# jchristopherson/nonlin

Measured on AMD Instinct MI355X. Metric: LM iterations/sec on m=4096,n=256 fp64; FD-Jacobian GB/s vs HBM peak, higher is better.
Workload: dtype f64

## Files before the change

### nonlin_amd/csrc/nlh_core.hip

```cpp
#include "nlh_internal.h"
#include "nlh_kernels_model.h"
#include "nlh_qrx.h"

int ensure(nlh_handle *h, DevBuf &b, size_t bytes)
{
    if (bytes <= b.bytes && b.p) return 0;
    if (b.p) { hipFree(b.p); b.p = nullptr; b.bytes = 0; }
    size_t want = bytes < 256 ? 256 : bytes;
    hipError_t e = hipMalloc(&b.p, want);
    if (e != hipSuccess) { h->err = std::string("hipMalloc: ") + hipGetErrorString(e); return NLH_OUT_OF_MEMORY_ERROR; }
    b.bytes = want;
    bool known = false;
    for (auto *q : h->bufs) if (q == &b) known = true;
    if (!known) h->bufs.push_back(&b);
    return 0;
}

bool lds_fits(const void *kernel, size_t dyn)
{
    static std::mutex mu;
    static std::vector<std::pair<const void *, size_t>> statics;
    size_t st = 0;
    {
        std::lock_guard<std::mutex> g(mu);
        auto it = std::find_if(statics.begin(), statics.end(), [&](const std::pair<const void *, size_t> &e) { return e.first == kernel; });
        if (it != statics.end()) st = it->second;
        else {
            hipFuncAttributes a;
            st = hipFuncGetAttributes(&a, kernel) == hipSuccess ? a.sharedSizeBytes : (size_t)NLH_LDS_MAX;
            statics.emplace_back(kernel, st);
        }
    }
    return st + dyn <= (size_t)NLH_LDS_MAX;
}

int ensure_staging(nlh_handle *h, size_t bytes)
{
    if (bytes <= h->staging_bytes) return 0;
    if (h->staging) hipHostFree(h->staging);
    h->staging = nullptr; h->staging_bytes = 0;
    if (hipHostMalloc(&h->staging, bytes, hipHostMallocDefault) != hipSuccess) { h->err = "hipHostMalloc (staging)"; return NLH_OUT_OF_MEMORY_ERROR; }
    h->staging_bytes = bytes;
    return 0;
}

int ensure_pinned(nlh_handle *h, size_t bytes)
{
    if (bytes <= h->pinned_bytes) return 0;
    if (h->pinned) hipHostFree(h->pinned);
    h->pinned = nullptr; h->pinned_bytes = 0;
    hipError_t e = hipHostMalloc(&h->pinned, bytes, hipHostMallocDefault);
    if (e != hipSuccess) { h->err = std::string("hipHostMalloc: ") + hipGetErrorString(e); return NLH_OUT_OF_MEMORY_ERROR; }
    h->pinned_bytes = bytes;
    return 0;
}

static const char *k_names[NLH_K_COUNT] = {
    "k_dq_residual", "k_dq_panel", "k_fd_jacobian", "k_gram_mfma", "k_gram_reduce", "k_jtf",
    "k_chol_factor", "k_lmpar", "k_qr_factor", "k_lm_update", "k_lu_factor", "k_dq_jacobian", "k_qrx_pass",
    "k_qrx_pivot", "k_polyroots", "k_covar"};

void timing_flush(nlh_handle *h)
{
    if (h->pending.empty()) return;
    hipStreamSynchronize(h->stream);
    for (auto &pr : h->pending) {
        float t = 0.f;
        if (hipEventElapsedTime(&t, pr.a, pr.b) == hipSuccess) h->ms[pr.kid] += (double)t;
        h->launches[pr.kid] += 1;
        if (pr.kid == h->sample_kid) h->samples.push_back(t);
        h->pool.push_back(pr.a);
        h->pool.push_back(pr.b);
    }
    h->pending.clear();
}

hipEvent_t ev_get(nlh_handle *h)
{
    if (!h->pool.empty()) { hipEvent_t e = h->pool.back(); h->pool.pop_back(); return e; }
    hipEvent_t e;
    hipEventCreate(&e);
    return e;
}
void nlh_default_options(nlh_options *o)
{
    o->max_evals = 100;
    o->ftol = 1.0e-8;
    o->xtol = 1.0e-12;
    o->gtol = 1.0e-12;
    o->print_status = 0;
    o->factor = 100.0;
    o->use_line_search = 1;
    o->ls_max_evals = 100;
    o->ls_alpha = 1.0e-4;
    o->ls_factor = 0.1;
    o->factor_policy = NLH_FACTOR_EXACT;
    o->ne_pivot_tol = 1.0e-4;
    o->fuse_fd = 1;
    o->sub_batches = 0;
}

int nlh_device_count(void)
{
    int n = 0;
    if (hipGetDeviceCount(&n) != hipSuccess) return 0;
    return n;
}

const char *nlh_version(void) { return "nonlin_hip 0.1 (gfx950)"; }

int nlh_create(nlh_handle **out, int32_t device, void *hip_stream)
{
    if (!out) return NLH_ERR_BAD_HANDLE;
    *out = nullptr;
    if (nlh_device_count() <= 0) return NLH_ERR_NO_DEVICE;
    if (hipSetDevice(device) != hipSuccess) return NLH_ERR_NO_DEVICE;
    nlh_handle *h = new nlh_handle();
    h->device = device;
    h->stream = (hipStream_t)hip_stream;
    const int lds_max = NLH_LDS_MAX;
    qrx_init_device();
    nlh_lm_init_device(lds_max);
    nlh_square_init_device(lds_max);
    nlh_cls_init_device(lds_max);
    nlh_bfgs_init_device(lds_max);
    nlh_poly_init_device(lds_max);
    nlh_polyroots_init_device(lds_max);
    nlh_covar_init_device(lds_max);
    nlh_devfcn_init_device(lds_max);
    nlh_expr_init_device(lds_max);
    (void)hipFuncSetAttribute((const void *)k_dq_residual<RB>, hipFuncAttributeMaxDynamicSharedMemorySize, lds_max);
    (void)hipFuncSetAttribute((const void *)k_dq_residual2<RB / 2>, hipFuncAttributeMaxDynamicSharedMemorySize, lds_max);
    (void)hipGetLastError();
    *out = h;
    return 0;
}

void nlh_destroy(nlh_handle *h)
{
    if (!h) return;
    for (auto *wk : h->workers) nlh_destroy(wk);
    h->workers.clear();
    hipSetDevice(h->device);
    hipStreamSynchronize(h->stream);
    timing_flush(h);
    for (auto e : h->pool) hipEventDestroy(e);
    for (auto *b : h->bufs) if (b->p) hipFree(b->p);
    if (h->pinned) hipHostFree(h->pinned);
    if (h->staging) hipHostFree(h->staging);
    if (h->lu_side) { hipStreamSynchronize(h->lu_side); hipStreamDestroy(h->lu_side); }
    if (h->lu_panel_done) hipEventDestroy(h->lu_panel_done);
    for (auto e : h->lu_bulk_done) if (e) hipEventDestroy(e);
    if (h->own_stream) hipStreamDestroy(h->stream);
    delete h;
}

const char *nlh_last_error(const nlh_handle *h) { return h ? h->err.c_str() : "null handle"; }

void nlh_timing_enable(nlh_handle *h, int32_t on)
{
    if (!h) return;
    h->timing = on == 0 ? 0u : on == 1 ? 0xffffffffu : ((uint32_t)on >> 1);
}
void nlh_timing_reset(nlh_handle *h)
{
    if (!h) return;
    timing_flush(h);
    for (int k = 0; k < NLH_K_COUNT; ++k) { h->ms[k] = 0; h->launches[k] = 0; }
    h->samples.clear();
}
int64_t nlh_timing_samples(nlh_handle *h, int32_t kid, float *out_ms, int64_t cap)
{
    if (!h) return NLH_ERR_BAD_HANDLE;
    if (kid != h->sample_kid) {
        timing_flush(h);
        h->sample_kid = kid;
        h->samples.clear();
        return 0;
    }
    timing_flush(h);
    const int64_t cnt = (int64_t)h->samples.size();
    for (int64_t i = 0; i < cnt && i < cap; ++i) out_ms[i] = h->samples[(size_t)i];
    return cnt;
}
int nlh_timing_get(nlh_handle *h, int32_t kid, double *total_ms, int64_t *launches)
{
    if (!h || kid < 0 || kid >= NLH_K_COUNT) return NLH_ERR_BAD_HANDLE;
    timing_flush(h);
    if (total_ms) *total_ms = h->ms[kid];
    if (launches) *launches = h->launches[kid];
    return 0;
}
const char *nlh_kernel_name(int32_t kid) { return (kid >= 0 && kid < NLH_K_COUNT) ? k_names[kid] : "?"; }




__device__ __forceinline__ double sm64_u(uint64_t seed, uint64_t k)
{
    uint64_t z = seed + (k + 1ULL) * 0x9E3779B97F4A7C15ULL;
    z = (z ^ (z >> 30)) * 0xBF58476D1CE4E5B9ULL;
    z = (z ^ (z >> 27)) * 0x94D049BB133111EBULL;
    z ^= z >> 31;
    return (double)(z >> 11) * 0x1.0p-53;
}

__global__ void k_gen_A(int m, int n, uint64_t seed0, uint64_t stride, int square_shift, double *A, double *xtrue)
{
    const int p = blockIdx.y;
    const uint64_t seed = seed0 + (uint64_t)p * stride;
    const size_t mn = (size_t)m * n;
    const double rs = sqrt((double)n);
    for (size_t e = (size_t)blockIdx.x * blockDim.x + threadIdx.x; e < mn + (size_t)n; e += (size_t)gridDim.x * blockDim.x) {
        const double u = 2.0 * sm64_u(seed, e) - 1.0;
        if (e < mn) {
            double v = u / rs;
            const size_t i = e % m, j = e / m;
            if (square_shift && i == j) v = 2.0 + v;
            A[(size_t)p * mn + e] = v;
        } else {
            xtrue[(size_t)p * n + (e - mn)] = u;
        }
    }
}

__global__ void k_gen_bx(int m, int n, uint64_t seed0, uint64_t stride, double sigma, double spread, double *b,
                         const double *xtrue, double *x0)
{
    const int p = blockIdx.y;
    const uint64_t seed = seed0 + (uint64_t)p * stride;
    const size_t base = (size_t)m * n + (size_t)n;
    for (size_t e = (size_t)blockIdx.x * blockDim.x + threadIdx.x; e < (size_t)m + n; e += (size_t)gridDim.x * blockDim.x) {
        const double u = 2.0 * sm64_u(seed, base + e) - 1.0;
        if (e < (size_t)m) b[(size_t)p * m + e] = b[(size_t)p * m + e] + sigma * u;
        else x0[(size_t)p * n + (e - m)] = xtrue[(size_t)p * n + (e - m)] + spread * u;
    }
}


void launch_dq_residual(nlh_handle *h, int nprob, int m, int n, const double *A, const double *b,
                               double gamma, const double *x, double *f, double *part,
                               const LmState *st, int want)
{
    Timed t(h, NLH_K_DQ_RESIDUAL);
    size_t sh = sizeof(double) * (size_t)(n + 32);
    const bool vec2 = (m % 2 == 0) && ((((uintptr_t)A | (uintptr_t)b | (uintptr_t)f) & 15) == 0);
    const int nblk = (m + RB - 1) / RB;
    for (int p0 = 0; p0 < nprob; p0 += NLH_MAX_LOCKSTEP) {
        const int cnt = std::min<int>(NLH_MAX_LOCKSTEP, nprob - p0);
        dim3 grid(nblk, cnt);
        const double *Ap = A + (size_t)p0 * m * n, *bp = b + (size_t)p0 * m, *xp = x + (size_t)p0 * n;
        double *fp = f + (size_t)p0 * m, *pp = part ? part + (size_t)p0 * nblk * 2 : nullptr;
        const LmState *sp = st ? st + p0 : nullptr;
        if (vec2)
            hipLaunchKernelGGL(k_dq_residual2<RB / 2>, grid, dim3(RB / 2), sh, h->stream, m, n, Ap, bp, gamma, xp, fp, pp, sp, want);
        else
            hipLaunchKernelGGL(k_dq_residual<RB>, grid, dim3(RB), sh, h->stream, m, n, Ap, bp, gamma, xp, fp, pp, sp, want);
    }
}

void launch_dq_panel(nlh_handle *h, int nprob, int m, int n, const double *A, const double *b,
                            double gamma, const double *x, double *P, const LmState *st, int want,
                            const double *f0_fused, bool to_qrx)
{
    Timed t(h, NLH_K_DQ_PANEL);
    constexpr int JT = 32;
    dim3 grid((m + RB - 1) / RB, (n + JT - 1) / JT, nprob);
    size_t sh = sizeof(double) * (size_t)n;
    const int tld = to_qrx ? qrx_ld(n) : 0, tcoff = to_qrx ? qrx_ld(n) - (n + 1) : 0;
    const size_t tst = to_qrx ? qrx_matrix_stride(m, n) : 0;
    if (f0_fused)
        hipLaunchKernelGGL((k_dq_panel<RB, JT, true>), grid, dim3(RB), sh, h->stream, m, n, A, b, gamma, x, P, f0_fused, st, want,
                           tld, tcoff, tst);
    else
        hipLaunchKernelGGL((k_dq_panel<RB, JT, false>), grid, dim3(RB), sh, h->stream, m, n, A, b, gamma, x, P,
                           (const double *)nullptr, st, want, 0, 0, (size_t)0);
}

void launch_fd(nlh_handle *h, int nprob, int m, int n, const double *P, const double *f0,
                      const double *x, double *J, const LmState *st, int want)
{
    Timed t(h, NLH_K_FD_JACOBIAN);
    constexpr int CJ = 8;
    const bool vec2 = (m % 2 == 0) && ((((uintptr_t)P | (uintptr_t)J | (uintptr_t)f0) & 15) == 0);
    if (vec2) {
        dim3 grid((m / 2 + RB - 1) / RB, (n + CJ - 1) / CJ, nprob);
        hipLaunchKernelGGL((k_fd_jacobian<RB, CJ, true>), grid, dim3(RB), 0, h->stream, m, n, P, f0, x, J, st, want);
    } else {
        dim3 grid((m + RB - 1) / RB, (n + CJ - 1) / CJ, nprob);
        hipLaunchKernelGGL((k_fd_jacobian<RB, CJ, false>), grid, dim3(RB), 0, h->stream, m, n, P, f0, x, J, st, want);
    }
}

void format_e10_3(double v, char out[16])
{
    char body[16];
    if (std::isnan(v)) { snprintf(out, 16, "%10s", "NaN"); return; }
    if (std::isinf(v)) { snprintf(out, 16, "%10s", v < 0 ? "-Inf" : "Inf"); return; }
    char sci[32];
    snprintf(sci, sizeof sci, "%.2e", fabs(v));
    int ex = atoi(sci + 5);
    if (v != 0.0) ex += 1;
    const char sign = std::signbit(v) && v != 0.0 ? '-' : ' ';
    if (abs(ex) < 100) snprintf(body, sizeof body, "%c0.%c%c%cE%c%02d", sign, sci[0], sci[2], sci[3], ex < 0 ? '-' : '+', abs(ex));
    else snprintf(body, sizeof body, "%c0.%c%c%c%c%03d", sign, sci[0], sci[2], sci[3], ex < 0 ? '-' : '+', abs(ex));
    snprintf(out, 16, "%10s", body);
}

void print_status(int iter, int nfeval, int njaceval, double xnorm, double fnorm)
{
    char a[16], b[16];
    format_e10_3(xnorm, a);
    format_e10_3(fnorm, b);
    printf(" \nIteration: %d\nFunction Evaluations: %d\n", iter, nfeval);
    if (njaceval > 0) printf("Jacobian Evaluations: %d\n", njaceval);
    printf("Change in Variable: %s\nResidual: %s\n", a, b);
    fflush(stdout);
}

int nlh_format_status(int32_t iter, int32_t nfeval, int32_t njaceval, double xnorm, double fnorm, char *buf,
                                 int32_t len)
{
    char a[16], b[16], jl[48] = "";
    format_e10_3(xnorm, a);
    format_e10_3(fnorm, b);
    if (njaceval > 0) snprintf(jl, sizeof jl, "Jacobian Evaluations: %d\n", njaceval);
    return snprintf(buf, len > 0 ? (size_t)len : 0, " \nIteration: %d\nFunction Evaluations: %d\n%sChange in Variable: %s\nResidual: %s\n",
                    iter, nfeval, jl, a, b);
}
int lockstep_slices(int32_t nprob, const std::function<int(int32_t, int32_t)> &run)
{
    for (int32_t p0 = 0; p0 < nprob; p0 += NLH_MAX_LOCKSTEP) {
        const int rc = run(p0, std::min<int32_t>(NLH_MAX_LOCKSTEP, nprob - p0));
        if (rc) return rc;
    }
    return 0;
}


int ensure_workers(nlh_handle *h, int T)
{
    while ((int)h->workers.size() < T) {
        nlh_handle *wk = new nlh_handle();
        wk->device = h->device;
        if (hipStreamCreateWithFlags(&wk->stream, hipStreamNonBlocking) != hipSuccess) { delete wk; h->err = "hipStreamCreate"; return NLH_ERR_HIP; }
        wk->own_stream = true;
        h->workers.push_back(wk);
    }
    return 0;
}

int run_problems(nlh_handle *h, int nprob, const std::function<int(nlh_handle *, int)> &solve_one)
{
    int T = 8;
    if (const char *e = getenv("NLH_WORKERS")) T = atoi(e);
    T = std::max(1, std::min(T, nprob));
    if (T == 1) {
        for (int p = 0; p < nprob; ++p) {
            const int rc = solve_one(h, p);
            if (rc != 0) return rc;
        }
        return 0;
    }
    { const int rcw = ensure_workers(h, T); if (rcw) return rcw; }
    HIPCHK(h, hipStreamSynchronize(h->stream));
    std::atomic<int> next(0), err(0);
    std::vector<std::thread> pool;
    for (int t = 0; t < T; ++t)
        pool.emplace_back([&, t]() {
            nlh_handle *wk = h->workers[t];
            if (hipSetDevice(wk->device) != hipSuccess) { err = NLH_ERR_HIP; return; }
            for (;;) {
                const int p = next.fetch_add(1);
                if (p >= nprob || err.load() != 0) break;
                const int rc = solve_one(wk, p);
                if (rc != 0) { err = rc; break; }
            }
            hipStreamSynchronize(wk->stream);
        });
    for (auto &th : pool) th.join();
    if (err.load() != 0) {
        for (auto *wk : h->workers) if (!wk->err.empty()) { h->err = wk->err; break; }
        return err.load();
    }
    return 0;
}

int nlh_dq_generate(nlh_handle *h, int32_t nprob, int32_t m, int32_t n, uint64_t seed0, uint64_t seed_stride, double gamma,
                    double sigma, double spread, int32_t square_shift, double *dA, double *db,
                    double *dxtrue, double *dx0)
{
    if (!h) return NLH_ERR_BAD_HANDLE;
    HIPCHK(h, hipSetDevice(h->device));
    const size_t mn = (size_t)m * n;
    unsigned gx = (unsigned)((mn + n + 255) / 256);
    if (gx > 4096) gx = 4096;
    hipLaunchKernelGGL(k_gen_A, dim3(gx, nprob), dim3(256), 0, h->stream, m, n, seed0, seed_stride, square_shift, dA, dxtrue);
    HIPCHK(h, hipMemsetAsync(db, 0, sizeof(double) * (size_t)nprob * m, h->stream));
    launch_dq_residual(h, nprob, m, n, dA, db, gamma, dxtrue, db, nullptr, nullptr, -1);
    unsigned gb = (unsigned)(((size_t)m + n + 255) / 256);
    hipLaunchKernelGGL(k_gen_bx, dim3(gb, nprob), dim3(256), 0, h->stream, m, n, seed0, seed_stride, sigma, spread, db, dxtrue, dx0);
    HIPCHK(h, hipGetLastError());
    return 0;
}

int nlh_dq_residual(nlh_handle *h, int32_t nprob, int32_t m, int32_t n, const double *dA, const double *db,
                    double gamma, const double *dx, double *df)
{
    if (!h) return NLH_ERR_BAD_HANDLE;
    HIPCHK(h, hipSetDevice(h->device));
    launch_dq_residual(h, nprob, m, n, dA, db, gamma, dx, df, nullptr, nullptr, -1);
    HIPCHK(h, hipGetLastError());
    return 0;
}

int nlh_dq_fd_panel(nlh_handle *h, int32_t nprob, int32_t m, int32_t n, const double *dA, const double *db,
                    double gamma, const double *dx, double *dP)
{
    if (!h) return NLH_ERR_BAD_HANDLE;
    if (m < 1 || n < 1) return NLH_INVALID_INPUT_ERROR;
    HIPCHK(h, hipSetDevice(h->device));
    launch_dq_panel(h, nprob, m, n, dA, db, gamma, dx, dP, nullptr, -1);
    HIPCHK(h, hipGetLastError());
    return 0;
}

int nlh_fd_jacobian_panel(nlh_handle *h, int32_t nprob, int32_t m, int32_t n, const double *dP,
                          const double *df0, const double *dx, double *dJ)
{
    if (!h) return NLH_ERR_BAD_HANDLE;
    HIPCHK(h, hipSetDevice(h->device));
    launch_fd(h, nprob, m, n, dP, df0, dx, dJ, nullptr, -1);
    HIPCHK(h, hipGetLastError());
    return 0;
}

int nlh_dq_jacobian(nlh_handle *h, int32_t nprob, int32_t m, int32_t n, const double *dA, double gamma,
                    const double *dx, double *dJ)
{
    if (!h) return NLH_ERR_BAD_HANDLE;
    HIPCHK(h, hipSetDevice(h->device));
    {
        Timed t(h, NLH_K_DQ_JACOBIAN);
        hipLaunchKernelGGL(k_dq_jacobian<RB>, dim3((m + RB - 1) / RB, nprob), dim3(RB), sizeof(double) * n, h->stream,
                           m, n, dA, gamma, dx, dJ, (const LmState *)nullptr, -1);
    }
    HIPCHK(h, hipGetLastError());
    return 0;
}
```

### nonlin_amd/csrc/nlh_kernels_model.h

```cpp
#pragma once
#include "nlh_common.h"

template <int BS>
__global__ void __launch_bounds__(BS)
k_dq_residual(int m, int n, const double *__restrict__ A, const double *__restrict__ b,
              double gamma, const double *__restrict__ xsrc, double *__restrict__ fout,
              double *__restrict__ part, const LmState *__restrict__ st, int want_stage)
{
    extern __shared__ double smem[];
    const int p = blockIdx.y;
    if (st && st[p].stage != want_stage) return;
    double *xs = smem;
    double *red = smem + n;
    const double *Ap = A + (size_t)p * m * n;
    const double *xp = xsrc + (size_t)p * n;
    for (int k = threadIdx.x; k < n; k += BS) xs[k] = xp[k];
    __syncthreads();

    const int i = blockIdx.x * BS + threadIdx.x;
    double r = 0.0;
    if (i < m) {
        double u = 0.0;
        const double *a = Ap + i;
        int k = 0;
        for (; k + 16 <= n; k += 16) {
            double av[16];
#pragma unroll
            for (int q = 0; q < 16; ++q) av[q] = a[(size_t)(k + q) * m];
#pragma unroll
            for (int q = 0; q < 16; ++q) u = u + av[q] * xs[k + q];
        }
        for (; k < n; ++k) u = u + a[(size_t)k * m] * xs[k];
        r = (u + (gamma * u) * u) - b[(size_t)p * m + i];
        fout[(size_t)p * m + i] = r;
    }
    if (part) {
        double sq = (i < m) ? r * r : 0.0;
        double tq = (i < m && i >= n) ? sq : 0.0;
        double s = block_reduce_sum(sq, red);
        double t = block_reduce_sum(tq, red);
        if (threadIdx.x == 0) {
            part[((size_t)p * gridDim.x + blockIdx.x) * 2 + 0] = s;
            part[((size_t)p * gridDim.x + blockIdx.x) * 2 + 1] = t;
        }
    }
}

template <int BS>
__global__ void __launch_bounds__(BS)
k_dq_residual2(int m, int n, const double *__restrict__ A, const double *__restrict__ b,
               double gamma, const double *__restrict__ xsrc, double *__restrict__ fout,
               double *__restrict__ part, const LmState *__restrict__ st, int want_stage)
{
    extern __shared__ double smem[];
    const int p = blockIdx.y;
    if (st && st[p].stage != want_stage) return;
    double *xs = smem;
    double *red = smem + n;
    const double *Ap = A + (size_t)p * m * n;
    const double *xp = xsrc + (size_t)p * n;
    for (int k = threadIdx.x; k < n; k += BS) xs[k] = xp[k];
    __syncthreads();

    const int i = (blockIdx.x * BS + threadIdx.x) * 2;
    double r0 = 0.0, r1 = 0.0;
    if (i < m) {
        double u0 = 0.0, u1 = 0.0;
        const double *a = Ap + i;
        int k = 0;
        for (; k + 16 <= n; k += 16) {
            double2 av[16];
#pragma unroll
            for (int q = 0; q < 16; ++q) av[q] = *reinterpret_cast<const double2 *>(a + (size_t)(k + q) * m);
#pragma unroll
            for (int q = 0; q < 16; ++q) {
                const double xk = xs[k + q];
                u0 = u0 + av[q].x * xk;
                u1 = u1 + av[q].y * xk;
            }
        }
        for (; k < n; ++k) {
            const double2 av = *reinterpret_cast<const double2 *>(a + (size_t)k * m);
            u0 = u0 + av.x * xs[k];
            u1 = u1 + av.y * xs[k];
        }
        const double2 bv = *reinterpret_cast<const double2 *>(b + (size_t)p * m + i);
        r0 = (u0 + (gamma * u0) * u0) - bv.x;
        r1 = (u1 + (gamma * u1) * u1) - bv.y;
        *reinterpret_cast<double2 *>(fout + (size_t)p * m + i) = make_double2(r0, r1);
    }
    if (part) {
        const double q0 = (i < m) ? r0 * r0 : 0.0, q1 = (i < m) ? r1 * r1 : 0.0;
        const double sq = q0 + q1;
        const double tq = ((i < m && i >= n) ? q0 : 0.0) + ((i < m && i + 1 >= n) ? q1 : 0.0);
        double s = block_reduce_sum(sq, red);
        double t = block_reduce_sum(tq, red);
        if (threadIdx.x == 0) {
            part[((size_t)p * gridDim.x + blockIdx.x) * 2 + 0] = s;
            part[((size_t)p * gridDim.x + blockIdx.x) * 2 + 1] = t;
        }
    }
}

template <int BS, int JT, bool FUSE>
__global__ void __launch_bounds__(BS)
k_dq_panel(int m, int n, const double *__restrict__ A, const double *__restrict__ b,
           double gamma, const double *__restrict__ x, double *__restrict__ P,
           const double *__restrict__ f0, const LmState *__restrict__ st, int want_stage,
           int tld, int tcoff, size_t tst)
{
    extern __shared__ double smem[];
    const int p = blockIdx.z;
    if (st && st[p].stage != want_stage) return;
    double *xs = smem;
    const double *Ap = A + (size_t)p * m * n;
    const double *xp = x + (size_t)p * n;
    for (int k = threadIdx.x; k < n; k += BS) xs[k] = xp[k];
    __syncthreads();

    const int j0 = blockIdx.y * JT;
    const int i = blockIdx.x * BS + threadIdx.x;
    if (i >= m) return;
    const int jt = min(JT, n - j0);
    const double *a = Ap + i;

    constexpr int PF = 8;
    double base = 0.0;
    {
        int k = 0;
        for (; k + PF <= j0; k += PF) {
            double av[PF];
#pragma unroll
            for (int u = 0; u < PF; ++u) av[u] = a[(size_t)(k + u) * m];
#pragma unroll
            for (int u = 0; u < PF; ++u) base = base + av[u] * xs[k + u];
        }
        for (; k < j0; ++k) base = base + a[(size_t)k * m] * xs[k];
    }

    double acc[JT];
#pragma unroll
    for (int jj = 0; jj < JT; ++jj) acc[jj] = base;

#pragma unroll
    for (int kk = 0; kk < JT; ++kk) {
        if (kk < jt) {
            const int k = j0 + kk;
            const double av = a[(size_t)k * m];
            const double xk = xs[k];
            const double pr = av * xk;
            const double pp = av * (xk + fd_step(xk));
#pragma unroll
            for (int jj = 0; jj < JT; ++jj) acc[jj] = acc[jj] + (jj == kk ? pp : pr);
        }
    }
    {
        int k = j0 + JT;
        double av[PF], aw[PF];
        if (k + PF <= n) {
#pragma unroll
            for (int u = 0; u < PF; ++u) av[u] = a[(size_t)(k + u) * m];
        }
        for (; k + PF <= n; k += PF) {
            const bool more = k + 2 * PF <= n;
            if (more) {
#pragma unroll
                for (int u = 0; u < PF; ++u) aw[u] = a[(size_t)(k + PF + u) * m];
            }
#pragma unroll
            for (int u = 0; u < PF; ++u) {
                const double pr = av[u] * xs[k + u];
#pragma unroll
                for (int jj = 0; jj < JT; ++jj) acc[jj] = acc[jj] + pr;
            }
            if (more) {
#pragma unroll
                for (int u = 0; u < PF; ++u) av[u] = aw[u];
            }
        }
        for (; k < n; ++k) {
            const double pr = a[(size_t)k * m] * xs[k];
#pragma unroll
            for (int jj = 0; jj < JT; ++jj) acc[jj] = acc[jj] + pr;
        }
    }
    const double bi = b[(size_t)p * m + i];
    const double f0i = FUSE ? f0[(size_t)p * m + i] : 0.0;
    double *Pp = tld ? P + (size_t)p * tst + ((size_t)(i >> 3) * tld + tcoff) * 8 + (i & 7) : P + (size_t)p * m * n + i;
    const size_t cstride = tld ? (size_t)8 : (size_t)m;
#pragma unroll
    for (int jj = 0; jj < JT; ++jj) {
        if (jj < jt) {
            const double u = acc[jj];
            const double r = (u + (gamma * u) * u) - bi;
            if (FUSE) __builtin_nontemporal_store((r - f0i) / fd_step(xs[j0 + jj]), Pp + (size_t)(j0 + jj) * cstride);
            else __builtin_nontemporal_store(r, Pp + (size_t)(j0 + jj) * cstride);
        }
    }
}

template <int BS, int CJ, bool VEC2>
__global__ void __launch_bounds__(BS)
k_fd_jacobian(int m, int n, const double *__restrict__ P, const double *__restrict__ f0,
              const double *__restrict__ x, double *__restrict__ J,
              const LmState *__restrict__ st, int want_stage, const int32_t *__restrict__ list = nullptr, int nfull = 0)
{
    const int p = list ? list[blockIdx.z] : blockIdx.z;
    if (st && st[p].stage != want_stage) return;
    const int ns = nfull ? nfull : n;
    const double *Pp = P + (size_t)blockIdx.z * m * n;
    double *Jp = J + (size_t)p * m * ns;
    const double *fp = f0 + (size_t)p * m;
    const double *xp = x + (size_t)p * ns;
    const int jbeg = blockIdx.y * CJ;
    const int jend = min(n, jbeg + CJ);
    if (VEC2) {
        const int i = (blockIdx.x * BS + threadIdx.x) * 2;
        if (i >= m) return;
        const double2 f = *reinterpret_cast<const double2 *>(fp + i);
#pragma unroll 4
        for (int j = jbeg; j < jend; ++j) {
            const double h = fd_step(xp[j]);
            typedef double v2d __attribute__((ext_vector_type(2)));
            const v2d v = __builtin_nontemporal_load(reinterpret_cast<const v2d *>(Pp + (size_t)j * m + i));
            v2d o;
            o.x = (v.x - f.x) / h;
            o.y = (v.y - f.y) / h;
            __builtin_nontemporal_store(o, reinterpret_cast<v2d *>(Jp + (size_t)j * m + i));
        }
    } else {
        const int i = blockIdx.x * BS + threadIdx.x;
        if (i >= m) return;
        const double f = fp[i];
        for (int j = jbeg; j < jend; ++j) {
            const double h = fd_step(xp[j]);
            Jp[(size_t)j * m + i] = (Pp[(size_t)j * m + i] - f) / h;
        }
    }
}

template <int BS>
__global__ void __launch_bounds__(BS)
k_dq_jacobian(int m, int n, const double *__restrict__ A, double gamma,
              const double *__restrict__ x, double *__restrict__ J, const LmState *__restrict__ st, int want)
{
    extern __shared__ double smem[];
    const int p = blockIdx.y;
    if (st && st[p].stage != want) return;
    double *xs = smem;
    const double *Ap = A + (size_t)p * m * n;
    const double *xp = x + (size_t)p * n;
    for (int k = threadIdx.x; k < n; k += BS) xs[k] = xp[k];
    __syncthreads();
    const int i = blockIdx.x * BS + threadIdx.x;
    if (i >= m) return;
    const double *a = Ap + i;
    double u = 0.0;
    for (int k = 0; k < n; ++k) u = u + a[(size_t)k * m] * xs[k];
    const double s = 1.0 + 2.0 * gamma * u;
    double *Jp = J + (size_t)p * m * n + i;
    for (int k = 0; k < n; ++k) Jp[(size_t)k * m] = s * a[(size_t)k * m];
}
```

Before: 3713.

## Replace dq_panel kernel with LDS-staged multi-wave row-tile kernel and prefix reuse

Adds k_dq_panel_rows, where each block covers a row tile with several waves handling different 32-column groups. A chunks are double-buffered through LDS with register prefetch and shared across those waves. A running prefix dot-product is reused, so the perturbed-column sums avoid recomputing the full product per column group. For the QRX-packed output layout, results are transposed through LDS so stores are vectorised. This aims to cut redundant global reads of A and uncoalesced panel stores, at the cost of more LDS, more barriers and higher register pressure from 32 accumulators.

Result: no change. 3724, median of 6 (+0.3%).

```diff
diff --git a/nonlin_amd/csrc/nlh_core.hip b/nonlin_amd/csrc/nlh_core.hip
--- a/nonlin_amd/csrc/nlh_core.hip
+++ b/nonlin_amd/csrc/nlh_core.hip
@@ -108,6 +108,13 @@
 }
 
 const char *nlh_version(void) { return "nonlin_hip 0.1 (gfx950)"; }
+
+template <int R, int G>
+static void dq_panel_rows_init(int lds_max)
+{
+    (void)hipFuncSetAttribute((const void *)k_dq_panel_rows<R, G, true>, hipFuncAttributeMaxDynamicSharedMemorySize, lds_max);
+    (void)hipFuncSetAttribute((const void *)k_dq_panel_rows<R, G, false>, hipFuncAttributeMaxDynamicSharedMemorySize, lds_max);
+}
 
 int nlh_create(nlh_handle **out, int32_t device, void *hip_stream)
 {
@@ -131,6 +138,10 @@
     nlh_expr_init_device(lds_max);
     (void)hipFuncSetAttribute((const void *)k_dq_residual<RB>, hipFuncAttributeMaxDynamicSharedMemorySize, lds_max);
     (void)hipFuncSetAttribute((const void *)k_dq_residual2<RB / 2>, hipFuncAttributeMaxDynamicSharedMemorySize, lds_max);
+    dq_panel_rows_init<64, 8>(lds_max);
+    dq_panel_rows_init<128, 4>(lds_max);
+    dq_panel_rows_init<256, 2>(lds_max);
+    dq_panel_rows_init<256, 1>(lds_max);
     (void)hipGetLastError();
     *out = h;
     return 0;
@@ -259,22 +270,40 @@
     }
 }
 
+template <int R, int G>
+static size_t dq_panel_rows_lds(int n, bool turn)
+{
+    const size_t stage = 2 * 1024, pieces = turn ? (size_t)(R * G / 64) * 8 * DQP_TURN_LD : 0;
+    return sizeof(double) * ((size_t)((n + 1) & ~1) + 2 * G * DQP_JT + std::max(stage, pieces));
+}
+
+template <int R, int G>
+static void dq_panel_rows(nlh_handle *h, int nprob, int m, int n, const double *A, const double *b, double gamma, const double *x,
+                          double *P, const LmState *st, int want, const double *f0, int tld, int tcoff, size_t tst)
+{
+    const int ntiles = (n + DQP_JT - 1) / DQP_JT;
+    dim3 grid((m + R - 1) / R, (ntiles + G - 1) / G, nprob);
+    const size_t sh = dq_panel_rows_lds<R, G>(n, tld > 0);
+    if (f0)
+        hipLaunchKernelGGL((k_dq_panel_rows<R, G, true>), grid, dim3(R * G), sh, h->stream, m, n, A, b, gamma, x, P, f0, st, want,
+                           tld, tcoff, tst);
+    else
+        hipLaunchKernelGGL((k_dq_panel_rows<R, G, false>), grid, dim3(R * G), sh, h->stream, m, n, A, b, gamma, x, P,
+                           (const double *)nullptr, st, want, tld, tcoff, tst);
+}
+
 void launch_dq_panel(nlh_handle *h, int nprob, int m, int n, const double *A, const double *b,
                             double gamma, const double *x, double *P, const LmState *st, int want,
                             const double *f0_fused, bool to_qrx)
 {
     Timed t(h, NLH_K_DQ_PANEL);
-    constexpr int JT = 32;
-    dim3 grid((m + RB - 1) / RB, (n + JT - 1) / JT, nprob);
-    size_t sh = sizeof(double) * (size_t)n;
     const int tld = to_qrx ? qrx_ld(n) : 0, tcoff = to_qrx ? qrx_ld(n) - (n + 1) : 0;
     const size_t tst = to_qrx ? qrx_matrix_stride(m, n) : 0;
-    if (f0_fused)
-        hipLaunchKernelGGL((k_dq_panel<RB, JT, true>), grid, dim3(RB), sh, h->stream, m, n, A, b, gamma, x, P, f0_fused, st, want,
-                           tld, tcoff, tst);
-    else
-        hipLaunchKernelGGL((k_dq_panel<RB, JT, false>), grid, dim3(RB), sh, h->stream, m, n, A, b, gamma, x, P,
-                           (const double *)nullptr, st, want, 0, 0, (size_t)0);
+    const int ntiles = (n + DQP_JT - 1) / DQP_JT;
+    if (ntiles > 4) dq_panel_rows<64, 8>(h, nprob, m, n, A, b, gamma, x, P, st, want, f0_fused, tld, tcoff, tst);
+    else if (ntiles > 2) dq_panel_rows<128, 4>(h, nprob, m, n, A, b, gamma, x, P, st, want, f0_fused, tld, tcoff, tst);
+    else if (ntiles > 1) dq_panel_rows<256, 2>(h, nprob, m, n, A, b, gamma, x, P, st, want, f0_fused, tld, tcoff, tst);
+    else dq_panel_rows<256, 1>(h, nprob, m, n, A, b, gamma, x, P, st, want, f0_fused, tld, tcoff, tst);
 }
 
 void launch_fd(nlh_handle *h, int nprob, int m, int n, const double *P, const double *f0,
diff --git a/nonlin_amd/csrc/nlh_kernels_model.h b/nonlin_amd/csrc/nlh_kernels_model.h
--- a/nonlin_amd/csrc/nlh_kernels_model.h
+++ b/nonlin_amd/csrc/nlh_kernels_model.h
@@ -196,6 +196,186 @@
             if (FUSE) __builtin_nontemporal_store((r - f0i) / fd_step(xs[j0 + jj]), Pp + (size_t)(j0 + jj) * cstride);
             else __builtin_nontemporal_store(r, Pp + (size_t)(j0 + jj) * cstride);
         }
+    }
+}
+
+#define DQP_JT 32
+#define DQP_TURN_LD (8 * 8 + 8)
+template <int R, int G, bool FUSE>
+__global__ void __launch_bounds__(R * G)
+k_dq_panel_rows(int m, int n, const double *__restrict__ A, const double *__restrict__ b,
+                double gamma, const double *__restrict__ x, double *__restrict__ P,
+                const double *__restrict__ f0, const LmState *__restrict__ st, int want_stage,
+                int tld, int tcoff, size_t tst)
+{
+    constexpr int JT = DQP_JT, NT = R * G, KC = 1024 / R, CH = KC * R, LPT = CH / 2 / NT;
+    static_assert(R % 64 == 0 && JT % KC == 0 && LPT >= 1 && LPT * 2 * NT == CH, "k_dq_panel_rows: shape");
+    typedef double v2d __attribute__((ext_vector_type(2)));
+    extern __shared__ __attribute__((aligned(16))) double dqp_smem[];
+    const int p = blockIdx.z;
+    if (st && st[p].stage != want_stage) return;
+    const int tid = threadIdx.x, lane = tid & 63, w = tid >> 6;
+    int rw, tg;
+    if (G == 8) { rw = 0; tg = w < 4 ? w : 11 - w; }
+    else if (G == 4) { rw = w >> 2; tg = rw ? 3 - (w & 3) : (w & 3); }
+    else if (G == 2) { rw = w >> 1; tg = ((w >> 2) ^ w) & 1; }
+    else { rw = w; tg = 0; }
+    const int i0 = blockIdx.x * R;
+    const int jg0 = blockIdx.y * (G * JT);
+    const int j0 = jg0 + tg * JT;
+    const bool active = j0 < n;
+    const int jt = min(JT, n - j0);
+    const int npad = (n + 1) & ~1;
+    double *xs = dqp_smem;
+    double *hs = xs + npad;
+    double *xhs = hs + G * JT;
+    double *stage = xhs + G * JT;
+    const double *Ap = A + (size_t)p * m * n;
+    const double *xp = x + (size_t)p * n;
+    for (int k = tid; k < n; k += NT) xs[k] = xp[k];
+    for (int c = tid; c < G * JT; c += NT) {
+        if (jg0 + c < n) {
+            const double xv = xp[jg0 + c];
+            const double h = fd_step(xv);
+            hs[c] = h;
+            xhs[c] = xv + h;
+        }
+    }
+
+    const bool vec2 = (m % 2 == 0) && (((uintptr_t)Ap & 15) == 0);
+    auto gload = [&](int c, v2d (&r)[LPT]) {
+#pragma unroll
+        for (int l = 0; l < LPT; ++l) {
+            const int q = tid + l * NT;
+            const int k = c * KC + q / (R / 2), i = i0 + 2 * (q % (R / 2));
+            r[l] = v2d{0.0, 0.0};
+            if (k < n) {
+                const double *src = Ap + (size_t)k * m + i;
+                if (vec2) {
+                    if (i < m) r[l] = *reinterpret_cast<const v2d *>(src);
+                } else {
+                    if (i < m) r[l].x = src[0];
+                    if (i + 1 < m) r[l].y = src[1];
+                }
+            }
+        }
+    };
+    const int nch = (n + KC - 1) / KC;
+    v2d ra[LPT], rb[LPT];
+    gload(0, ra);
+    gload(1, rb);
+
+    double acc[JT];
+#pragma unroll
+    for (int jj = 0; jj < JT; ++jj) acc[jj] = 0.0;
+    double run = 0.0;
+    for (int c = 0; c < nch; ++c) {
+        double *buf = stage + (c & 1) * CH;
+#pragma unroll
+        for (int l = 0; l < LPT; ++l) {
+            const int q = tid + l * NT;
+            *reinterpret_cast<v2d *>(buf + (q / (R / 2)) * R + 2 * (q % (R / 2))) = ra[l];
+        }
+#pragma unroll
+        for (int l = 0; l < LPT; ++l) ra[l] = rb[l];
+        gload(c + 2, rb);
+        nlh_lds_barrier();
+        if (!active) continue;
+        const int k0 = c * KC;
+        const double *arow = buf + rw * 64 + lane;
+        if (k0 + KC <= j0) {
+#pragma unroll
+            for (int u = 0; u < KC; ++u) run = run + arow[u * R] * xs[k0 + u];
+        } else if (k0 >= j0 + JT) {
+            if (k0 + KC <= n) {
+#pragma unroll
+                for (int u = 0; u < KC; ++u) {
+                    const double pr = arow[u * R] * xs[k0 + u];
+#pragma unroll
+                    for (int jj = 0; jj < JT; ++jj) acc[jj] = acc[jj] + pr;
+                }
+            } else {
+#pragma unroll
+                for (int u = 0; u < KC; ++u) {
+                    if (k0 + u < n) {
+                        const double pr = arow[u * R] * xs[k0 + u];
+#pragma unroll
+                        for (int jj = 0; jj < JT; ++jj) acc[jj] = acc[jj] + pr;
+                    }
+                }
+            }
+        } else {
+#pragma unroll
+            for (int s = 0; s < JT / KC; ++s) {
+                if (k0 - j0 == s * KC) {
+#pragma unroll
+                    for (int u = 0; u < KC; ++u) {
+                        const int kk = s * KC + u;
+                        if (kk < jt) {
+                            const double av = arow[u * R];
+                            const double pr = av * xs[k0 + u];
+                            const double pp = av * xhs[tg * JT + kk];
+                            acc[kk] = run + pp;
+#pragma unroll
+                            for (int jj = 0; jj < kk; ++jj) acc[jj] = acc[jj] + pr;
+                            run = run + pr;
+                        }
+                    }
+                }
+            }
+        }
+    }
+
+    const int i = i0 + rw * 64 + lane;
+    const double bi = i < m ? b[(size_t)p * m + i] : 0.0;
+    const double f0i = (FUSE && i < m) ? f0[(size_t)p * m + i] : 0.0;
+    if (!tld) {
+        if (active && i < m) {
+            double *Pp = P + (size_t)p * m * n + i;
+#pragma unroll
+            for (int jj = 0; jj < JT; ++jj) {
+                if (jj < jt) {
+                    const double u = acc[jj];
+                    const double r = (u + (gamma * u) * u) - bi;
+                    if (FUSE) __builtin_nontemporal_store((r - f0i) / hs[tg * JT + jj], Pp + (size_t)(j0 + jj) * m);
+                    else __builtin_nontemporal_store(r, Pp + (size_t)(j0 + jj) * m);
+                }
+            }
+        }
+        return;
+    }
+    double *Tp = P + (size_t)p * tst;
+    double *tw = stage + w * (8 * DQP_TURN_LD);
+    nlh_lds_barrier();
+#pragma unroll
+    for (int pc = 0; pc < JT / 8; ++pc) {
+        if (active) {
+#pragma unroll
+            for (int c = 0; c < 8; ++c) {
+                const int jj = pc * 8 + c;
+                if (jj < jt) {
+                    const double u = acc[jj];
+                    const double r = (u + (gamma * u) * u) - bi;
+                    tw[(lane >> 3) * DQP_TURN_LD + c * 8 + (lane & 7)] = FUSE ? (r - f0i) / hs[tg * JT + jj] : r;
+                }
+            }
+        }
+        nlh_lds_barrier();
+        if (active) {
+#pragma unroll
+            for (int it = 0; it < 4; ++it) {
+                const int q = it * 64 + lane;
+                const int rbk = q >> 5, wi = q & 31;
+                const int ii = i0 + rw * 64 + rbk * 8 + (wi & 3) * 2;
+                if (pc * 8 + (wi >> 2) < jt && ii < m) {
+                    const v2d o = *reinterpret_cast<const v2d *>(tw + rbk * DQP_TURN_LD + wi * 2);
+                    double *dst = Tp + ((size_t)(ii >> 3) * tld + tcoff + j0 + pc * 8) * 8 + wi * 2;
+                    if (ii + 1 < m) __builtin_nontemporal_store(o, reinterpret_cast<v2d *>(dst));
+                    else __builtin_nontemporal_store(o.x, dst);
+                }
+            }
+        }
+        nlh_lds_barrier();
     }
 }
 
diff --git a/profiles/dq_panel_callers.py b/profiles/dq_panel_callers.py
--- /dev/null
+++ b/profiles/dq_panel_callers.py
@@ -0,0 +1,94 @@
+#!/usr/bin/env python3
+import json
+import os
+import statistics
+import sys
+import time
+
+ROOT = os.path.dirname(os.path.dirname(os.path.abspath(__file__)))
+sys.path.insert(0, ROOT)
+
+
+def main():
+    from nonlin_amd import _lib
+    args = sys.argv[1:]
+    if "--lib" in args:
+        _lib.LIB_PATH = os.path.abspath(args[args.index("--lib") + 1])
+    import numpy as np
+    import torch
+    from nonlin_amd.device import DeviceSolver
+    ds = DeviceSolver(0)
+    out = {"lib": _lib.LIB_PATH}
+    if "--solvers" in args:
+        xg = [None]
+
+        def timed(f, reps=5):
+            f()
+            torch.cuda.synchronize()
+            ts = []
+            for _ in range(reps):
+                t0 = time.perf_counter()
+                f()
+                torch.cuda.synchronize()
+                ts.append(round(1e3 * (time.perf_counter() - t0), 3))
+            return ts
+
+        def cls(nb, m, n, **gen):
+            A, b, xt, x0 = ds.generate(nb, m, n, seed0=12345, **gen)
+            lo, up = np.full(n, -2.0), np.full(n, 2.0)
+
+            def run():
+                xg[0] = x0.clone()
+                return ds.cls_solve_batch(A, b, 0.5, xg[0], opts=ds.options(max_evals=500), lower=lo, upper=up)
+            return timed(run)
+
+        def bfgs(nb, m, n):
+            A, b, xt, x0 = ds.generate(nb, m, n, seed0=77, spread=0.1)
+
+            def run():
+                xg[0] = x0.clone()
+                return ds.bfgs_solve_batch(A, b, 0.5, xg[0], opts=ds.options(max_evals=400, gtol=1e-8, xtol=1e-12))
+            return timed(run)
+
+        def newton_fd(n):
+            A, b, xt, x0 = ds.generate(1, n, n, seed0=12345, sigma=0.0, square_shift=True)
+
+            def run():
+                xg[0] = x0.clone()
+                return ds.newton_solve_batch(A, b, 0.5, xg[0], analytic=False, opts=ds.options(max_evals=500))
+            return timed(run)
+
+        out["cls_1x4096x256_ms"] = cls(1, 4096, 256)
+        out["cls_256x2048x128_ms"] = cls(256, 2048, 128, spread=0.2)
+        out["bfgs_1x2048x256_ms"] = bfgs(1, 2048, 256)
+        out["bfgs_256x1024x64_ms"] = bfgs(256, 1024, 64)
+        out["newton_fd_1x1024_ms"] = newton_fd(1024)
+    else:
+        ds.h.timing_enable(kernels=["dq_panel"])
+        ds.h.timing_samples("dq_panel", select_only=True)
+        for (nprob, m, n) in [(1, 21, 4), (4096, 2048, 24), (1, 1024, 1024), (1, 65536, 512), (1024, 2048, 128)]:
+            A, b, xt, x0 = ds.generate(nprob, m, n, square_shift=(m == n))
+            P = ds.fd_panel(A, b, 0.5, x0)
+            torch.cuda.synchronize()
+            ds.h.timing_reset()
+            for _ in range(7):
+                P = ds.fd_panel(A, b, 0.5, x0)
+            torch.cuda.synchronize()
+            s = ds.h.timing_samples("dq_panel")
+            out[f"panel_{nprob}x{m}x{n}_ms"] = {"min": round(min(s), 4), "median": round(statistics.median(s), 4)}
+            del A, b, P
+            torch.cuda.empty_cache()
+        A, b, xt, x0 = ds.generate(2048, 4096, 256)
+        x = x0.clone()
+        ds.lm_solve_batch(A, b, 0.5, x, ds.options(max_evals=1, factor_policy=2))
+        torch.cuda.synchronize()
+        ds.h.timing_reset()
+        x = x0.clone()
+        ds.lm_solve_batch(A, b, 0.5, x, ds.options(max_evals=3, factor_policy=2))
+        torch.cuda.synchronize()
+        out["lm_fused_2048x4096x256_ms"] = [round(v, 3) for v in ds.h.timing_samples("dq_panel")]
+    print(json.dumps(out), flush=True)
+
+
+if __name__ == "__main__":
+    main()
```
